# CliMA/OrthogonalSphericalShellGrids.jl

Measured on AMD Instinct MI355X. Metric: grid-cells/s metric precompute + zipper halo-fill GB/s, 1/10°×75z, higher is better.
Workload: dtype f64

## Files before the change

### orthogonalsphericalshellgrids.jl_amd/csrc/tpg_grid.hip

```cpp
#include "tpg_common.hpp"
#include "tpg_math.hpp"
#include "tpg_batch.hpp"

using namespace tpgm;

namespace {

constexpr double kC180Pi = 180.0 / kPi;
constexpr double kC360Pi = 360.0 / kPi;

struct GridK {
    int Nx, Ny, Hx, Hy;
    int shift;
    int jstart, jend;
    int jm_lo, jm_hi;
    int sx, rows;
    int ft;
    double fplp90;
    double R;
    const double* ti;
    const double* tj;
    const double* ts;
};

struct OutPtrs { void* p[TPG_NUM_ARRAYS]; };

struct TableArgs {
    int Nx, Ny, Hy, shift, ft;
    double south, npl, R;
    double* ti; double* tj; double* ts;
};

__device__ double lambda_face(int i, int N, int ft)
{
    long long num = 360ll * (i - 1) - 180ll * N;
    if (ft == TPG_F32) return (double)((float)num / (float)N);
    return (double)num / (double)N;
}
__device__ double lambda_center(int i, int N, int ft)
{
    long long num = 360ll * (2ll * i - 1) - 360ll * N;
    if (ft == TPG_F32) return (double)((float)num / (float)(2ll * N));
    return (double)num / (double)(2ll * N);
}
__device__ double phi_center(int j, int N, double south)
{
    if (N == 1) return south;
    if (south == __builtin_rint(south) && absD(south) < 1e6) {
        long long s = (long long)south;
        long long num = s * (N - 1) + (90 - s) * (long long)(j - 1);
        return (double)num / (double)(N - 1);
    }
    dd step = dd_div(two_sum(90.0, -south), dd{ (double)(N - 1), 0.0 });
    dd v = dd_add(dd{ south, 0.0 }, dd_mul_d(step, (double)(j - 1)));
    return v.hi + v.lo;
}

__global__ __launch_bounds__(64) void k_tables(TableArgs t)
{
    int tid = blockIdx.x * blockDim.x + threadIdx.x;
    const double a = tand((90.0 - t.npl) / 2);
    if (tid < t.Nx) {
        int is = tid + 1;
        int i0 = is - t.shift; if (i0 < 1) i0 += t.Nx;
        double lf = lambda_face(i0, t.Nx, t.ft), lc = lambda_center(i0, t.Nx, t.ft);
        double slf = sind(lf), clf = cosd(lf), slc = sind(lc), clc = cosd(lc);
        if (t.ft == TPG_F32) {
            slf = (double)(float)slf; clf = (double)(float)clf; slc = (double)(float)slc; clc = (double)(float)clc;
        }
        t.ti[0 * t.Nx + tid] = a * slf;
        t.ti[1 * t.Nx + tid] = a * clf;
        t.ti[2 * t.Nx + tid] = a * slc;
        t.ti[3 * t.Nx + tid] = a * clc;
        return;
    }
    tid -= t.Nx;
    if (tid < 2 * t.Ny) {
        int face = tid < t.Ny;
        int j = (face ? tid : tid - t.Ny) + 1;
        double pc = phi_center(j, t.Ny, t.south);
        double phi = pc;
        if (face) {
            double dphi = t.Ny > 1 ? phi_center(2, t.Ny, t.south) - phi_center(1, t.Ny, t.south) : 0.0;
            phi = pc - dphi / 2;
        }
        double psi = asinhD(tand((90.0 - phi) / 2) / a);
        double sh, ch;
        sinh_cosh(psi, sh, ch);
        int base = face ? 0 : 2;
        t.tj[(base + 0) * t.Ny + (j - 1)] = sh;
        t.tj[(base + 1) * t.Ny + (j - 1)] = ch;
        return;
    }
    tid -= 2 * t.Ny;
    if (tid <= t.Hy) {
        int j = 1 - t.Hy + tid;
        const double south = t.south, R = t.R;
        const double dlam = 360.0 / (double)t.Nx;
        const double dphiL = (90.0 - south) / (double)t.Ny;
        double pf, pfn, pc, pcm;
        if (south == __builtin_rint(south)) {
            long long s = (long long)south, Ny = t.Ny;
            pf  = (double)(s * Ny + (90 - s) * (long long)(j - 1)) / (double)Ny;
            pfn = (double)(s * Ny + (90 - s) * (long long)j) / (double)Ny;
            pc  = (double)(2 * s * Ny + (90 - s) * (long long)(2 * j - 1)) / (double)(2 * Ny);
            pcm = (double)(2 * s * Ny + (90 - s) * (long long)(2 * j - 3)) / (double)(2 * Ny);
        } else {
            pf  = south + (double)(j - 1) * dphiL;
            pfn = south + (double)j * dphiL;
            pc  = south + ((double)(2 * j - 1) * (90.0 - south)) / (double)(2 * t.Ny);
            pcm = south + ((double)(2 * j - 3) * (90.0 - south)) / (double)(2 * t.Ny);
        }
        int n = t.Hy + 1;
        t.ts[0 * n + tid] = R * (dlam * kDeg2Rad) * cosD(kPi * pc / 180);
        t.ts[1 * n + tid] = R * (dlam * kDeg2Rad) * cosD(kPi * pf / 180);
        t.ts[2 * n + tid] = R * R * (dlam * kDeg2Rad) * (sinD(kPi * pfn / 180) - sinD(kPi * pf / 180));
        t.ts[3 * n + tid] = R * R * (dlam * kDeg2Rad) * (sinD(kPi * pc / 180) - sinD(kPi * pcm / 180));
        t.ts[4 * n + tid] = R * (dphiL * kDeg2Rad);
    }
}

struct LP { double lam, phi; };

__device__ __forceinline__ LP analytic(const GridK& g, int xl, int yl, int is, int js)
{
    int i0 = is - g.shift; if (i0 < 1) i0 += g.Nx;
    const double* ti = g.ti + (xl == TPG_FACE ? 0 : 2) * g.Nx;
    const double* tj = g.tj + (yl == TPG_FACE ? 0 : 2) * g.Ny;
    double asl = ti[is - 1], acl = ti[g.Nx + is - 1];
    double sh = tj[js - 1], ch = tj[g.Ny + js - 1];
    double x = asl * ch;
    double y = acl * sh;
    bool pole = (x == 0.0) & (y == 0.0);
    double l = pole ? (i0 == 1 ? -90.0 : 90.0) : -kC180Pi * atanD(y / x);
    LP r;
    r.phi = 90.0 - kC360Pi * atanD(sqrt(y * y + x * x));
    l += (i0 <= g.Nx / 2) ? -90.0 : 90.0;
    l += g.fplp90;
    r.lam = fmod360(fmod360(l) + 360.0);
    return r;
}

__device__ __forceinline__ int fold_partner(int xl, int i, int Nx)
{
    int ip = (xl == TPG_FACE) ? Nx - i + 2 : Nx - i + 1;
    return ip > Nx ? ip - Nx : ip;
}

__device__ __forceinline__ LP coord(const GridK& g, int xl, int yl, int i, int j)
{
    if (j < 1) return LP{ 0.0, 0.0 };
    int iw = i < 1 ? i + g.Nx : (i > g.Nx ? i - g.Nx : i);
    int js = j;
    if (j > g.Ny) {
        int dj = j - g.Ny;
        js = (yl == TPG_FACE) ? g.Ny - dj + 1 : g.Ny - dj;
        iw = fold_partner(xl, iw, g.Nx);
        if (js < 1) return LP{ 0.0, 0.0 };
    } else if (j == g.Ny && yl == TPG_CENTER && iw > g.Nx / 2) {
        iw = fold_partner(xl, iw, g.Nx);
    }
    return analytic(g, xl, yl, iw, js);
}

__device__ __forceinline__ double haversine(LP a, LP b, double R)
{
    double dl = (b.lam - a.lam) * kDeg2Rad;
    double a1 = a.phi * kDeg2Rad;
    double a2 = b.phi * kDeg2Rad;
    double dp = a2 - a1;
    double s1 = sinD(dp / 2), s2 = sinD(dl / 2);
    double h = s1 * s1 + cosD(a1) * cosD(a2) * (s2 * s2);
    double r = sqrt(h);
    return 2 * (R * asinD(r != r ? r : (r < 1.0 ? r : 1.0)));
}

struct V3 { double x, y, z; };
__device__ __forceinline__ V3 cartesian(LP p)
{
    double cl = cosd(p.phi);
    return V3{ cosd(p.lam) * cl, sind(p.lam) * cl, sind(p.phi) };
}
__device__ __forceinline__ double dot3(V3 a, V3 b) { return a.x * b.x + a.y * b.y + a.z * b.z; }
__device__ __forceinline__ V3 cross3(V3 a, V3 b)
{
    return V3{ a.y * b.z - a.z * b.y, a.z * b.x - a.x * b.z, a.x * b.y - a.y * b.x };
}
__device__ __forceinline__ double tri_area(V3 a, V3 b, V3 c)
{
    double t = absD(dot3(a, cross3(b, c)));
    t /= 1 + dot3(a, b) + dot3(b, c) + dot3(a, c);
    return 2 * atanD(t);
}
__device__ __forceinline__ double quad_area(V3 a, V3 b, V3 c, V3 d)
{
    double A = tri_area(a, b, c);
    A += tri_area(a, b, d);
    A += tri_area(a, c, d);
    A += tri_area(b, c, d);
    return A / 2;
}

__device__ __forceinline__ double tri_tan_nr(V3 a, V3 b, V3 c)
{
    return div_nr(absD(dot3(a, cross3(b, c))), 1 + dot3(a, b) + dot3(b, c) + dot3(a, c));
}
__device__ __forceinline__ double tri_tan(V3 a, V3 b, V3 c)
{
    return absD(dot3(a, cross3(b, c))) / (1 + dot3(a, b) + dot3(b, c) + dot3(a, c));
}

template <typename T, bool NT = false>
__device__ __forceinline__ void put(const OutPtrs& o, int q, long long off, double v)
{
    T* p = static_cast<T*>(o.p[q]) + off;
    if (NT) __builtin_nontemporal_store((T)v, p); else *p = (T)v;
}

template <typename T, bool NT = false>
__device__ __forceinline__ void put32(const OutPtrs& o, int q, unsigned boff, double v)
{
    asm volatile("" : "+v"(boff));
    T* p = reinterpret_cast<T*>(static_cast<char*>(o.p[q]) + boff);
    if (NT) __builtin_nontemporal_store((T)v, p); else *p = (T)v;
}

template <typename T, bool NT>
__global__ __launch_bounds__(256) void k_cells(GridK g, OutPtrs o)
{
    const int nbx = (g.Nx + 255) / 256;
    int rb = blockIdx.x / nbx;
    int i = (blockIdx.x - rb * nbx) * 256 + threadIdx.x + 1;
    int j = g.jm_lo + rb;
    if (i > g.Nx) return;

    LP cc = coord(g, 0, 0, i, j), fc = coord(g, 1, 0, i, j), cf = coord(g, 0, 1, i, j), ff = coord(g, 1, 1, i, j);
    LP fc_e = coord(g, 1, 0, i + 1, j), fc_s = coord(g, 1, 0, i, j - 1);
    LP cc_w = coord(g, 0, 0, i - 1, j), cc_s = coord(g, 0, 0, i, j - 1), cc_sw = coord(g, 0, 0, i - 1, j - 1);
    LP ff_e = coord(g, 1, 1, i + 1, j), ff_n = coord(g, 1, 1, i, j + 1), ff_ne = coord(g, 1, 1, i + 1, j + 1);
    LP cf_w = coord(g, 0, 1, i - 1, j), cf_n = coord(g, 0, 1, i, j + 1);

    const double R = g.R;
    double dxcc = haversine(fc_e, fc, R);
    double dxfc = haversine(cc, cc_w, R);
    double dxcf = haversine(ff_e, ff, R);
    double dxff = haversine(cf, cf_w, R);
    double dycc = haversine(cf_n, cf, R);
    double dyfc = haversine(ff_n, ff, R);
    double dycf = haversine(cc, cc_s, R);
    double dyff = haversine(fc, fc_s, R);
    double azcc = quad_area(cartesian(ff), cartesian(ff_e), cartesian(ff_ne), cartesian(ff_n)) * (R * R);
    double azfc = dyfc * dxfc;
    double azcf = dycf * dxcf;
    double azff = quad_area(cartesian(cc_sw), cartesian(cc_s), cartesian(cc), cartesian(cc_w)) * (R * R);

    long long off = (long long)(i + g.Hx - 1) + (long long)g.sx * (j - g.jstart + g.Hy);
    put<T, NT>(o, TPG_LAMBDA_CC, off, cc.lam); put<T, NT>(o, TPG_LAMBDA_FC, off, fc.lam);
    put<T, NT>(o, TPG_LAMBDA_CF, off, cf.lam); put<T, NT>(o, TPG_LAMBDA_FF, off, ff.lam);
    put<T, NT>(o, TPG_PHI_CC, off, cc.phi); put<T, NT>(o, TPG_PHI_FC, off, fc.phi);
    put<T, NT>(o, TPG_PHI_CF, off, cf.phi); put<T, NT>(o, TPG_PHI_FF, off, ff.phi);
    put<T, NT>(o, TPG_DX_CC, off, dxcc); put<T, NT>(o, TPG_DX_FC, off, dxfc);
    put<T, NT>(o, TPG_DX_CF, off, dxcf); put<T, NT>(o, TPG_DX_FF, off, dxff);
    put<T, NT>(o, TPG_DY_CC, off, dycc); put<T, NT>(o, TPG_DY_CF, off, dycf);
    put<T, NT>(o, TPG_DY_FC, off, dyfc); put<T, NT>(o, TPG_DY_FF, off, dyff);
    put<T, NT>(o, TPG_AZ_CC, off, azcc); put<T, NT>(o, TPG_AZ_FC, off, azfc);
    put<T, NT>(o, TPG_AZ_CF, off, azcf); put<T, NT>(o, TPG_AZ_FF, off, azff);
}

struct Pt  { double lam, phi, a, ca; };
struct PtX { double lam, phi, a, ca, X, Y, Z; };
struct Nb  { double lam, a, ca; };
struct NbX { double lam, a, ca, X, Y, Z; };

__device__ __forceinline__ Pt make_pt(const GridK& g, int xl, int yl, int i, int j)
{
    LP p = coord(g, xl, yl, i, j);
    Pt r; r.lam = p.lam; r.phi = p.phi; r.a = p.phi * kDeg2Rad; r.ca = cosD(r.a);
    return r;
}
__device__ __forceinline__ PtX make_ptx(const GridK& g, int xl, int yl, int i, int j)
{
    LP p = coord(g, xl, yl, i, j);
    PtX r; r.lam = p.lam; r.phi = p.phi; r.a = p.phi * kDeg2Rad; r.ca = cosD(r.a);
    double sl, cl, sp, cp;
    sincosd(p.lam, sl, cl);
    sincosd(p.phi, sp, cp);
    r.X = cl * cp; r.Y = sl * cp; r.Z = sp;
    return r;
}
__device__ __forceinline__ Nb nb_of(const Pt& p) { return Nb{ p.lam, p.a, p.ca }; }
__device__ __forceinline__ Nb nb_of(const PtX& p) { return Nb{ p.lam, p.a, p.ca }; }
__device__ __forceinline__ NbX nbx_of(const PtX& p) { return NbX{ p.lam, p.a, p.ca, p.X, p.Y, p.Z }; }
__device__ __forceinline__ V3 v3_of(const PtX& p) { return V3{ p.X, p.Y, p.Z }; }
__device__ __forceinline__ V3 v3_of(const NbX& p) { return V3{ p.X, p.Y, p.Z }; }

template <int DIR> __device__ __forceinline__ double shf(double v)
{
    return DIR > 0 ? __shfl_down(v, 1, 64) : __shfl_up(v, 1, 64);
}
template <int DIR> __device__ __forceinline__ Nb shf_nb(const Pt& p)
{
    return Nb{ shf<DIR>(p.lam), shf<DIR>(p.a), shf<DIR>(p.ca) };
}
template <int DIR> __device__ __forceinline__ NbX shf_nbx(const PtX& p)
{
    return NbX{ shf<DIR>(p.lam), shf<DIR>(p.a), shf<DIR>(p.ca), shf<DIR>(p.X), shf<DIR>(p.Y), shf<DIR>(p.Z) };
}

__device__ __forceinline__ double hav(double xlam, double xa, double xca, double ylam, double ya, double yca, double R)
{
    double dl = (ylam - xlam) * kDeg2Rad;
    double dp = ya - xa;
    double s1 = sinD(dp / 2), s2 = sinD(dl / 2);
    double h = s1 * s1 + xca * yca * (s2 * s2);
    double r = sqrt(h);
    return 2 * (R * asinD(r != r ? r : (r < 1.0 ? r : 1.0)));
}
#define HAV(P, Q) hav((P).lam, (P).a, (P).ca, (Q).lam, (Q).a, (Q).ca, R)


struct Step4 {
    double lam[4], phi[4], a[4], ca[4];
    double X[2], Y[2], Z[2];
};

struct LaneConst { double aslF, aclF, aslC, aclC, hemi; };

struct RowTab { double shC, chC, shF, chF; };

typedef const double __attribute__((address_space(4))) kconst_double;
__device__ __forceinline__ RowTab load_rowtab(const GridK& g, int jc, int jf)
{
    kconst_double* tj = (kconst_double*)g.tj;
    jc = __builtin_amdgcn_readfirstlane(jc < 1 ? 1 : (jc > g.Ny ? g.Ny : jc));
    jf = __builtin_amdgcn_readfirstlane(jf < 1 ? 1 : (jf > g.Ny ? g.Ny : jf));
    return RowTab{ tj[2 * g.Ny + jc - 1], tj[3 * g.Ny + jc - 1], tj[0 * g.Ny + jf - 1], tj[1 * g.Ny + jf - 1] };
}

__device__ __forceinline__ void points_fast(const GridK& g, const LaneConst& lc, const RowTab& rt, Step4& s, const double* atab)
{
    const double shC = rt.shC, chC = rt.chC, shF = rt.shF, chF = rt.chF;
    double x[4] = { lc.aslF * chC, lc.aslC * chC, lc.aslF * chF, lc.aslC * chF };
    double y[4] = { lc.aclF * shC, lc.aclC * shC, lc.aclF * shF, lc.aclC * shF };
    double q[4], rr[4], at1[4], at2[4];
#pragma unroll
    for (int k = 0; k < 4; ++k) { q[k] = y[k] / x[k]; rr[k] = sqrt_nr<true>(y[k] * y[k] + x[k] * x[k]);    }
    tpgb::atan_tab_b<4>(q, at1, atab);
    tpgb::atan_tab_b<4, true>(rr, at2, atab);
#pragma unroll
    for (int k = 0; k < 4; ++k) {
        double l = -kC180Pi * at1[k];
        s.phi[k] = 90.0 - kC360Pi * at2[k];
        l += lc.hemi;
        l += g.fplp90;
        s.lam[k] = tpgb::fmod360_pos(tpgb::fmod360_small(l) + 360.0);
        s.a[k] = s.phi[k] * kDeg2Rad;
    }
    if (tpgb::cos_b<4>(s.a, s.ca)) {
#pragma unroll
        for (int k = 0; k < 4; ++k) s.ca[k] = cosD(s.a[k]);
    }
    double ang[4] = { s.lam[1], s.phi[1], s.lam[2], s.phi[2] }, sn[4], cs[4];
    tpgb::sincosd_b<4>(ang, sn, cs);
    s.X[0] = cs[0] * cs[1]; s.Y[0] = sn[0] * cs[1]; s.Z[0] = sn[1];
    s.X[1] = cs[2] * cs[3]; s.Y[1] = sn[2] * cs[3]; s.Z[1] = sn[3];
}

__device__ __forceinline__ void points_fast2(const GridK& g, const LaneConst& lc, const RowTab& rt, Step4& s, const double* atab)
{
    const double shC = rt.shC, chC = rt.chC, shF = rt.shF, chF = rt.chF;
    double x[4] = { lc.aslF * chC, lc.aslC * chC, lc.aslF * chF, lc.aslC * chF };
    double y[4] = { lc.aclF * shC, lc.aclC * shC, lc.aclF * shF, lc.aclC * shF };
    double q[4], rr[4], at1[4], at2[4];
    bool zerox = false;
#pragma unroll
    for (int k = 0; k < 4; ++k) { q[k] = div_nr(y[k], x[k]); zerox |= x[k] == 0.0; rr[k] = sqrt_nr<true>(y[k] * y[k] + x[k] * x[k]);    }
#pragma unroll
    for (int h = 0; h < 4; h += 2) {
        double qa[2] = { q[h], q[h + 1] }, ra[2] = { rr[h], rr[h + 1] }, o1[2], o2[2];
        tpgb::atan_tab_b<2, true>(qa, o1, atab);
        tpgb::atan_tab_b<2, true>(ra, o2, atab);
        at1[h] = o1[0]; at1[h + 1] = o1[1]; at2[h] = o2[0]; at2[h + 1] = o2[1];
    }
    if (zerox) {
#pragma unroll
        for (int k = 0; k < 4; ++k)
            if (x[k] == 0.0) {
                const double qq = y[k] / x[k];
                at1[k] = (qq != qq) ? qq : csign(kPio2Hi, qq);
            }
    }
#pragma unroll
    for (int k = 0; k < 4; ++k) {
        double l = -kC180Pi * at1[k];
        s.phi[k] = 90.0 - kC360Pi * at2[k];
        l += lc.hemi;
        l += g.fplp90;
        s.lam[k] = tpgb::fmod360_pos(tpgb::fmod360_small(l) + 360.0);
        s.a[k] = s.phi[k] * kDeg2Rad;
    }
    double sn[4], cs[4];
#pragma unroll
    for (int h = 0; h < 4; h += 2) {
        double aa[2] = { s.a[h], s.a[h + 1] }, cc2[2];
        if (tpgb::cos_lat_b<2>(aa, cc2)) { cc2[0] = cosD(aa[0]); cc2[1] = cosD(aa[1]); }
        s.ca[h] = cc2[0]; s.ca[h + 1] = cc2[1];
    }
    {
        double lon[2] = { s.lam[1], s.lam[2] }, lat[2] = { s.phi[1], s.phi[2] }, sl[2], cl[2], sp[2], cp[2];
        tpgb::sincosd_b<2>(lon, sl, cl);
        if (tpgb::sincosd_lat_b<2>(lat, sp, cp)) tpgb::sincosd_b<2>(lat, sp, cp);
        sn[0] = sl[0]; cs[0] = cl[0]; sn[1] = sp[0]; cs[1] = cp[0];
        sn[2] = sl[1]; cs[2] = cl[1]; sn[3] = sp[1]; cs[3] = cp[1];
    }
    s.X[0] = cs[0] * cs[1]; s.Y[0] = sn[0] * cs[1]; s.Z[0] = sn[1];
    s.X[1] = cs[2] * cs[3]; s.Y[1] = sn[2] * cs[3]; s.Z[1] = sn[3];
}

__device__ __noinline__ void points_general(const GridK& g, int i, int jc, int jf, Step4& s)
{
    Pt fc = make_pt(g, 1, 0, i, jc), cf = make_pt(g, 0, 1, i, jf);
    PtX cc = make_ptx(g, 0, 0, i, jc), ff = make_ptx(g, 1, 1, i, jf);
    s.lam[0] = fc.lam; s.phi[0] = fc.phi; s.a[0] = fc.a; s.ca[0] = fc.ca;
    s.lam[1] = cc.lam; s.phi[1] = cc.phi; s.a[1] = cc.a; s.ca[1] = cc.ca;
    s.lam[2] = ff.lam; s.phi[2] = ff.phi; s.a[2] = ff.a; s.ca[2] = ff.ca;
    s.lam[3] = cf.lam; s.phi[3] = cf.phi; s.a[3] = cf.a; s.ca[3] = cf.ca;
    s.X[0] = cc.X; s.Y[0] = cc.Y; s.Z[0] = cc.Z;
    s.X[1] = ff.X; s.Y[1] = ff.Y; s.Z[1] = ff.Z;
}

template <int R> struct TileLds { double v[18][R][64]; };
enum { L_FC = 0, L_CC = 3, L_FF = 9, L_CF = 15 };

template <int N>
__device__ __forceinline__ void hav_batch(const Nb (&X)[N], const Nb (&Y)[N], double Rad, double (&d)[N])
{
    double hp[N], hl[N], s1[N], s2[N], hh[N], rt[N], rm[N], as[N];
    bool zero = false;
#pragma unroll
    for (int e = 0; e < N; ++e) {
        double dp = Y[e].a - X[e].a;
        hp[e] = dp / 2; hl[e] = (Y[e].lam - X[e].lam) * (kDeg2Rad * 0.5);
    }
    if (tpgb::sin_small_b<N>(hp, s1)) {
#pragma unroll
        for (int e = 0; e < N; ++e) s1[e] = sinD(hp[e]);
    }
    if (tpgb::sin_small_b<N>(hl, s2)) {
#pragma unroll
        for (int e = 0; e < N; ++e) s2[e] = sinD(hl[e]);
    }
#pragma unroll
    for (int e = 0; e < N; ++e) {
        double h = s1[e] * s1[e] + X[e].ca * Y[e].ca * (s2[e] * s2[e]);
        hh[e] = h;
        zero |= h == 0.0;
        rt[e] = sqrt_nr<true>(h);
    }
    if (zero) {
#pragma unroll
        for (int e = 0; e < N; ++e) rt[e] = sqrt_nr(hh[e]);
    }
#pragma unroll
    for (int e = 0; e < N; ++e) {
        rm[e] = __builtin_fmin(rt[e], 1.0);
    }
    if (tpgb::asin_small_b<N>(rm, as)) {
#pragma unroll
        for (int e = 0; e < N; ++e) as[e] = asinD(!(rt[e] >= 1.0) ? rt[e] : 1.0);
    }
#pragma unroll
    for (int e = 0; e < N; ++e) d[e] = (2 * Rad) * as[e];
}

template <typename T, bool NT, int R>
__global__ __launch_bounds__(64 * R, 4) void k_cells_tile(GridK g, OutPtrs o, int tiles_x)
{
    __shared__ __attribute__((aligned(16))) double atabs[R][TPG_ATAN_TABLE_DOUBLES];
    __shared__ TileLds<R> lds;
    const int lane = threadIdx.x & 63;
    const int p = __builtin_amdgcn_readfirstlane(threadIdx.x >> 6);
    double* atab = atabs[p];
    tpgb::atan_table_init(atab, lane);
    __builtin_amdgcn_fence(__ATOMIC_RELEASE, "wavefront");
    __builtin_amdgcn_wave_barrier();
    __builtin_amdgcn_fence(__ATOMIC_ACQUIRE, "wavefront");
    const int ty = (int)gridDim.y - 1 - (int)blockIdx.y;
    const int tx = blockIdx.x;
    const int s0 = g.jm_lo - 1 + ty * (R - 1);
    const int s = s0 + p;
    int i = tx * 62 + lane;
    const bool col_emit = lane >= 1 && lane <= 62 && i <= g.Nx;
    if (i > g.Nx + 1) i = g.Nx + 1;
    const double Rad = g.R;
    const bool active_row = s <= g.jm_hi;
    const unsigned col = (unsigned)(i + g.Hx - 1);
    auto rowoff = [&](int j) -> unsigned { return (col + (unsigned)g.sx * (unsigned)(j - g.jstart + g.Hy)) * (unsigned)sizeof(T); };

    Step4 q;
    if (active_row) {
        const bool fast = s >= 1 && s < g.Ny && absD(g.fplp90) <= 360.0;
        if (fast) {
            LaneConst lc;
            const int iw = i < 1 ? i + g.Nx : (i > g.Nx ? i - g.Nx : i);
            int i0 = iw - g.shift; if (i0 < 1) i0 += g.Nx;
            lc.aslF = g.ti[0 * g.Nx + iw - 1]; lc.aclF = g.ti[1 * g.Nx + iw - 1];
            lc.aslC = g.ti[2 * g.Nx + iw - 1]; lc.aclC = g.ti[3 * g.Nx + iw - 1];
            lc.hemi = (i0 <= g.Nx / 2) ? -90.0 : 90.0;
            points_fast2(g, lc, load_rowtab(g, s, s + 1), q, atab);
        } else {
            Step4 tmp; GridK gc = g; points_general(gc, i, s, s + 1, tmp); q = tmp;
        }
        if (col_emit) {
            if (p >= 1 && s >= g.jm_lo) {
                unsigned off = rowoff(s);
                put32<T, NT>(o, TPG_LAMBDA_FC, off, q.lam[0]); put32<T, NT>(o, TPG_PHI_FC, off, q.phi[0]);
                put32<T, NT>(o, TPG_LAMBDA_CC, off, q.lam[1]); put32<T, NT>(o, TPG_PHI_CC, off, q.phi[1]);
            }
            if ((p >= 1 || ty == 0) && s + 1 >= g.jm_lo && s + 1 <= g.jm_hi) {
                unsigned off1 = rowoff(s + 1);
                put32<T, NT>(o, TPG_LAMBDA_FF, off1, q.lam[2]); put32<T, NT>(o, TPG_PHI_FF, off1, q.phi[2]);
                put32<T, NT>(o, TPG_LAMBDA_CF, off1, q.lam[3]); put32<T, NT>(o, TPG_PHI_CF, off1, q.phi[3]);
            }
        }
        double (*L)[R][64] = lds.v;
        L[L_FC + 0][p][lane] = q.lam[0]; L[L_FC + 1][p][lane] = q.a[0]; L[L_FC + 2][p][lane] = q.ca[0];
        L[L_CC + 0][p][lane] = q.lam[1]; L[L_CC + 1][p][lane] = q.a[1]; L[L_CC + 2][p][lane] = q.ca[1];
        L[L_CC + 3][p][lane] = q.X[0];   L[L_CC + 4][p][lane] = q.Y[0]; L[L_CC + 5][p][lane] = q.Z[0];
        L[L_FF + 0][p][lane] = q.lam[2]; L[L_FF + 1][p][lane] = q.a[2]; L[L_FF + 2][p][lane] = q.ca[2];
        L[L_FF + 3][p][lane] = q.X[1];   L[L_FF + 4][p][lane] = q.Y[1]; L[L_FF + 5][p][lane] = q.Z[1];
        L[L_CF + 0][p][lane] = q.lam[3]; L[L_CF + 1][p][lane] = q.a[3]; L[L_CF + 2][p][lane] = q.ca[3];
    }
    __syncthreads();
    if (p == 0) {
        if (!col_emit) return;
        double (*L)[R][64] = lds.v;
#pragma unroll 1
        for (int r = 1; r < R; r += 2) {
            const int sa = s0 + r, sb = sa + 1;
            if (sa > g.jm_hi) break;
            const bool two = (r + 1 < R) && sb <= g.jm_hi;
            const int rb = two ? r + 1 : r;
            Nb X[2] = { Nb{ L[L_FC + 0][r][lane], L[L_FC + 1][r][lane], L[L_FC + 2][r][lane] },
                        Nb{ L[L_FC + 0][rb][lane], L[L_FC + 1][rb][lane], L[L_FC + 2][rb][lane] } };
            Nb Y[2] = { Nb{ L[L_FC + 0][r - 1][lane], L[L_FC + 1][r - 1][lane], L[L_FC + 2][r - 1][lane] },
                        Nb{ L[L_FC + 0][rb - 1][lane], L[L_FC + 1][rb - 1][lane], L[L_FC + 2][rb - 1][lane] } };
            double dd2[2];
            hav_batch<2>(X, Y, Rad, dd2);
            if (sa >= g.jm_lo) put32<T, NT>(o, TPG_DY_FF, rowoff(sa), dd2[0]);
            if (two && sb >= g.jm_lo) put32<T, NT>(o, TPG_DY_FF, rowoff(sb), dd2[1]);
        }
        return;
    }
    if (!active_row || s < g.jm_lo || !col_emit) return;

    double (*L)[R][64] = lds.v;
    const int pm = p - 1, le = lane + 1, lw = lane - 1;
    const unsigned off = rowoff(s);

#pragma unroll
    for (int k = 0; k < 2; ++k) {
        V3 a, b, c, dd;
        if (k == 0) {
            a = V3{ L[L_FF + 3][pm][lane], L[L_FF + 4][pm][lane], L[L_FF + 5][pm][lane] };
            b = V3{ L[L_FF + 3][pm][le], L[L_FF + 4][pm][le], L[L_FF + 5][pm][le] };
            c = V3{ L[L_FF + 3][p][le], L[L_FF + 4][p][le], L[L_FF + 5][p][le] };
            dd = V3{ q.X[1], q.Y[1], q.Z[1] };
        } else {
            a = V3{ L[L_CC + 3][pm][lw], L[L_CC + 4][pm][lw], L[L_CC + 5][pm][lw] };
            b = V3{ L[L_CC + 3][pm][lane], L[L_CC + 4][pm][lane], L[L_CC + 5][pm][lane] };
            c = V3{ q.X[0], q.Y[0], q.Z[0] };
            dd = V3{ L[L_CC + 3][p][lw], L[L_CC + 4][p][lw], L[L_CC + 5][p][lw] };
        }
        double tt[4], at[4];
        tt[0] = tri_tan_nr(a, b, c); tt[1] = tri_tan_nr(a, b, dd);
        tt[2] = tri_tan_nr(a, c, dd); tt[3] = tri_tan_nr(b, c, dd);
        if (__any(tpgb::atan_small_b<4>(tt, at))) {
            tt[0] = tri_tan(a, b, c); tt[1] = tri_tan(a, b, dd); tt[2] = tri_tan(a, c, dd); tt[3] = tri_tan(b, c, dd);
            tpgb::atan_b<4>(tt, at);
        }
        double A = at[0];
        A += at[1];
        A += at[2];
        A += at[3];
        put32<T, NT>(o, k == 0 ? TPG_AZ_CC : TPG_AZ_FF, off, A * (Rad * Rad));
    }

    auto ld = [&](int f, int pp, int ll) -> Nb { return Nb{ L[f + 0][pp][ll], L[f + 1][pp][ll], L[f + 2][pp][ll] }; };
    const Nb own[4] = { Nb{ q.lam[0], q.a[0], q.ca[0] }, Nb{ q.lam[1], q.a[1], q.ca[1] },
                        Nb{ q.lam[2], q.a[2], q.ca[2] }, Nb{ q.lam[3], q.a[3], q.ca[3] } };
    double d[8];
#pragma unroll
    for (int hb = 0; hb < 6; hb += 2) {
        Nb X[2], Y[2];
        if (hb == 0)      { X[0] = ld(L_FC, p, le); Y[0] = own[0];            X[1] = own[1];            Y[1] = ld(L_CC, p, lw); }
        else if (hb == 2) { X[0] = ld(L_FF, pm, le); Y[0] = ld(L_FF, pm, lane); X[1] = ld(L_CF, pm, lane); Y[1] = ld(L_CF, pm, lw); }
        else              { X[0] = own[3];           Y[0] = ld(L_CF, pm, lane); X[1] = own[2];            Y[1] = ld(L_FF, pm, lane); }
        double dd2[2];
        hav_batch<2>(X, Y, Rad, dd2);
        d[hb] = dd2[0]; d[hb + 1] = dd2[1];
    }
    {
        Nb X[1] = { own[1] }, Y[1] = { ld(L_CC, pm, lane) };
        double dd1[1];
        hav_batch<1>(X, Y, Rad, dd1);
        d[6] = dd1[0];
    }
    put32<T, NT>(o, TPG_DX_CC, off, d[0]); put32<T, NT>(o, TPG_DX_FC, off, d[1]);
    put32<T, NT>(o, TPG_DX_CF, off, d[2]); put32<T, NT>(o, TPG_DX_FF, off, d[3]);
    put32<T, NT>(o, TPG_DY_CC, off, d[4]); put32<T, NT>(o, TPG_DY_FC, off, d[5]);
    put32<T, NT>(o, TPG_DY_CF, off, d[6]);
    put32<T, NT>(o, TPG_AZ_FC, off, d[5] * d[1]);
    put32<T, NT>(o, TPG_AZ_CF, off, d[6] * d[2]);
}

__device__ __forceinline__ void array_loc(int q, int& xl, int& yl)
{
    int r = q & 3;
    bool dy = (q >= TPG_DY_CC && q <= TPG_DY_FF);
    int xr = dy ? (r >> 1) : (r & 1);
    int yr = dy ? (r & 1) : (r >> 1);
    xl = xr; yl = yr;
}

struct HaloRegions {
    int nA;
    int nB;
    int nC;
    int nD;
    int nsouth;
    int merged_south;
};

template <typename T>
__global__ __launch_bounds__(256) void k_halos(GridK g, OutPtrs o, HaloRegions h)
{
    int t = blockIdx.x * blockDim.x + threadIdx.x;
    int q = blockIdx.y;
    int xl, yl;
    array_loc(q, xl, yl);
    const bool is_coord = q < TPG_DX_CC;
    T* A = static_cast<T*>(o.p[q]);
    const long long sx = g.sx;
    auto at = [&](int i, int j) -> long long { return (long long)(i + g.Hx - 1) + sx * (j - g.jstart + g.Hy); };

    int i, j;
    if (t < h.nA) {
        int r = t / (2 * g.Hx), c = t - r * 2 * g.Hx;
        j = g.jm_lo + r;
        i = c < g.Hx ? 1 - g.Hx + c : g.Nx + 1 + (c - g.Hx);
        if (h.merged_south && !is_coord && j <= 1) return;
    } else if ((t -= h.nA) < h.nB) {
        int r = t / g.sx, c = t - r * g.sx;
        j = g.Ny + 1 + r; i = 1 - g.Hx + c;
    } else if ((t -= h.nB) < h.nC) {
        int r = t / g.sx, c = t - r * g.sx;
        j = 1 - h.nsouth + r; i = 1 - g.Hx + c;
        if (is_coord) { if (j < 1) A[at(i, j)] = (T)0; return; }
        if (!h.merged_south) return;
        const int n = g.Hy + 1, rt = j - (1 - g.Hy);
        const int col = (q >= TPG_DY_CC && q <= TPG_DY_FF) ? 4 : ((q >= TPG_AZ_CC ? 2 : 0) + (yl == TPG_FACE ? 1 : 0));
        A[at(i, j)] = (T)g.ts[col * n + rt];
        return;
    } else if ((t -= h.nC) < h.nD) {
        if (is_coord || yl != TPG_CENTER) return;
        i = g.Nx / 2 + 1 + t; j = g.Ny;
    } else {
        return;
    }

    int iw = i < 1 ? i + g.Nx : (i > g.Nx ? i - g.Nx : i);
    int js = j;
    if (j > g.Ny) {
        int dj = j - g.Ny;
        js = (yl == TPG_FACE) ? g.Ny - dj + 1 : g.Ny - dj;
        iw = fold_partner(xl, iw, g.Nx);
        if (js < 1) { A[at(i, j)] = (T)0; return; }
    } else if (j == g.Ny && yl == TPG_CENTER && iw > g.Nx / 2) {
        iw = fold_partner(xl, iw, g.Nx);
    }
    A[at(i, j)] = A[at(iw, js)];
}

template <typename T>
__global__ __launch_bounds__(256) void k_south(GridK g, OutPtrs o)
{
    int c = blockIdx.x * blockDim.x + threadIdx.x;
    int r = blockIdx.y;
    int lr = (1 - g.Hy + r) - (g.jstart - g.Hy);
    if (c >= g.sx || lr < 0 || lr >= g.rows) return;
    int n = g.Hy + 1;
    double dxc = g.ts[0 * n + r], dxf = g.ts[1 * n + r], azc = g.ts[2 * n + r], azf = g.ts[3 * n + r], dy = g.ts[4 * n + r];
    long long off = (long long)c + (long long)g.sx * lr;
    put<T>(o, TPG_DX_FF, off, dxf); put<T>(o, TPG_DX_FC, off, dxc); put<T>(o, TPG_DX_CF, off, dxf); put<T>(o, TPG_DX_CC, off, dxc);
    put<T>(o, TPG_DY_FF, off, dy);  put<T>(o, TPG_DY_FC, off, dy);  put<T>(o, TPG_DY_CF, off, dy);  put<T>(o, TPG_DY_CC, off, dy);
    put<T>(o, TPG_AZ_FF, off, azf); put<T>(o, TPG_AZ_FC, off, azc); put<T>(o, TPG_AZ_CF, off, azf); put<T>(o, TPG_AZ_CC, off, azc);
}

size_t table_doubles(const tpg_params* p) { return 4 * (size_t)p->Nx + 4 * (size_t)p->Ny + 5 * (size_t)(p->Hy + 1); }

int check_params(const tpg_params* p)
{
    if (!p) { tpg::set_error("null params"); return TPG_ERR_INVALID_ARGUMENT; }
    int rc = tpg::check_geom(p->Nx, p->Ny, p->Nz, p->Hx, p->Hy, p->Hz, p->ft);
    if (rc) return rc;
    if (p->jstart < 1 || p->jend > p->Ny || p->jend < p->jstart) {
        tpg::set_error("latitude band %d:%d outside 1:%d", p->jstart, p->jend, p->Ny);
        return TPG_ERR_BAD_PARTITION;
    }
    if (p->reserved & ~TPG_BUILD_TABLES_VALID) {
        tpg::set_error("tpg_params.reserved: unknown flag bits 0x%x", p->reserved & ~TPG_BUILD_TABLES_VALID);
        return TPG_ERR_INVALID_ARGUMENT;
    }
    if (!(p->radius > 0) || !(p->north_poles_latitude < 90) || !(p->southernmost_latitude < 90)) {
        tpg::set_error("invalid radius / latitudes");
        return TPG_ERR_INVALID_ARGUMENT;
    }
    return TPG_OK;
}

template <typename T>
int launch_build(const GridK& g, const OutPtrs& o, const HaloRegions& h, hipStream_t s)
{
    dim3 grid1(((g.Nx + 255) / 256) * (g.jm_hi - g.jm_lo + 1));
    const tpg::Config& cfg = tpg::config();
    const bool nt = cfg.build_nt;
    constexpr int R = 8;
    const int nrows = g.jm_hi - g.jm_lo + 1;
    const int tiles_y = (nrows + (R - 1) - 1) / (R - 1);
    const bool offsets32 = (unsigned long long)g.sx * (unsigned long long)(g.jend - g.jstart + 1 + 2 * g.Hy) * sizeof(T) < (1ull << 32);
    const bool south_in_band = g.jstart - g.Hy <= 1;
    const bool tile = cfg.cells_variant != 0 && tiles_y <= 65535 && offsets32;
    if (tile) {
        const int tiles_x = (g.Nx + 61) / 62;
        dim3 gridt((unsigned)tiles_x, (unsigned)tiles_y);
        if (nt) hipLaunchKernelGGL((k_cells_tile<T, true, R>), gridt, dim3(64 * R), 0, s, g, o, tiles_x);
        else    hipLaunchKernelGGL((k_cells_tile<T, false, R>), gridt, dim3(64 * R), 0, s, g, o, tiles_x);
    }
    else if (nt) hipLaunchKernelGGL((k_cells<T, true>), grid1, dim3(256), 0, s, g, o);
    else         hipLaunchKernelGGL((k_cells<T, false>), grid1, dim3(256), 0, s, g, o);
    int rc = tpg::launch_status("k_cells");
    if (rc) return rc;
    HaloRegions hm = h;
    hm.merged_south = (south_in_band && g.Ny > 2 * g.Hy + 2) ? 1 : 0;
    if (hm.merged_south) hm.nC = (h.nsouth + 1) * g.sx;
    int nh = hm.nA + hm.nB + hm.nC + hm.nD;
    if (nh > 0) {
        hipLaunchKernelGGL(k_halos<T>, dim3((nh + 255) / 256, TPG_NUM_ARRAYS), dim3(256), 0, s, g, o, hm);
        if ((rc = tpg::launch_status("k_halos"))) return rc;
    }
    if (south_in_band && !hm.merged_south) {
        hipLaunchKernelGGL(k_south<T>, dim3((g.sx + 255) / 256, g.Hy + 1), dim3(256), 0, s, g, o);
        if ((rc = tpg::launch_status("k_south"))) return rc;
    }
    return TPG_OK;
}

}

extern "C" {

size_t tpg_build_grid_workspace_bytes(const tpg_params* p)
{
    if (!p || p->Nx < 1 || p->Ny < 1 || p->Hy < 0) return 0;
    return (table_doubles(p) * sizeof(double) + 255) & ~(size_t)255;
}

int tpg_build_grid(const tpg_params* p, void* const out[TPG_NUM_ARRAYS], void* workspace,
                   size_t workspace_bytes, void* stream)
{
    int rc = check_params(p);
    if (rc) return rc;
    if (!out) { tpg::set_error("null output table"); return TPG_ERR_INVALID_ARGUMENT; }
    OutPtrs o;
    for (int q = 0; q < TPG_NUM_ARRAYS; ++q) {
        if (!out[q]) { tpg::set_error("null output array %d", q); return TPG_ERR_INVALID_ARGUMENT; }
        o.p[q] = out[q];
    }
    if (!workspace || workspace_bytes < table_doubles(p) * sizeof(double) || ((uintptr_t)workspace & 7)) {
        tpg::set_error("workspace: need %zu bytes, 8-byte aligned", table_doubles(p) * sizeof(double));
        return TPG_ERR_WORKSPACE;
    }
    hipStream_t s = tpg::as_stream(stream);
    double* w = static_cast<double*>(workspace);

    TableArgs t;
    t.Nx = p->Nx; t.Ny = p->Ny; t.Hy = p->Hy; t.shift = p->Nx / 4; t.ft = p->ft;
    t.south = p->southernmost_latitude; t.npl = p->north_poles_latitude; t.R = p->radius;
    t.ti = w; t.tj = w + 4 * (size_t)p->Nx; t.ts = t.tj + 4 * (size_t)p->Ny;
    if (!(p->reserved & TPG_BUILD_TABLES_VALID)) {
        int nt = p->Nx + 2 * p->Ny + p->Hy + 1;
        hipLaunchKernelGGL(k_tables, dim3((nt + 63) / 64), dim3(64), 0, s, t);
        if ((rc = tpg::launch_status("k_tables"))) return rc;
    }

    GridK g;
    g.Nx = p->Nx; g.Ny = p->Ny; g.Hx = p->Hx; g.Hy = p->Hy; g.shift = p->Nx / 4;
    g.jstart = p->jstart; g.jend = p->jend;
    g.jm_lo = p->jstart - p->Hy < 1 ? 1 : p->jstart - p->Hy;
    g.jm_hi = p->jend + p->Hy > p->Ny ? p->Ny : p->jend + p->Hy;
    g.sx = p->Nx + 2 * p->Hx; g.rows = p->jend - p->jstart + 1 + 2 * p->Hy;
    g.ft = p->ft; g.fplp90 = p->first_pole_longitude + 90.0; g.R = p->radius;
    g.ti = t.ti; g.tj = t.tj; g.ts = t.ts;

    HaloRegions h;
    h.nA = (g.jm_hi - g.jm_lo + 1) * 2 * g.Hx;
    h.nB = (p->jend + p->Hy > p->Ny) ? (p->jend + p->Hy - p->Ny) * g.sx : 0;
    h.nsouth = (1 - (p->jstart - p->Hy)) > 0 ? (1 - (p->jstart - p->Hy)) : 0;
    h.nC = h.nsouth * g.sx;
    h.nD = (p->jend + p->Hy >= p->Ny) ? p->Nx / 2 : 0;

    if (p->ft == TPG_F64) return launch_build<double>(g, o, h, s);
    return launch_build<float>(g, o, h, s);
}

}
```

Before: 12.26 billion.

## Exploit tripolar grid mirror symmetry to halve atan and sincos work via wave shuffles

The tile kernel now assigns the lower half-wave to columns starting at a0 and the upper half-wave to the mirrored columns across the fold. Each lane computes the atan, cos and sincos for only its own row (C or F) and obtains the other row's values from its mirror lane via __shfl, with a sign fix on the longitude atan. The grid now covers only half of Nx. This roughly halves the expensive transcendental work per point, at the cost of shuffles, more complex indexing and wrapping, extra LDS reads, and reliance on the grid being exactly symmetric.

```diff
diff --git a/orthogonalsphericalshellgrids.jl_amd/csrc/tpg_grid.hip b/orthogonalsphericalshellgrids.jl_amd/csrc/tpg_grid.hip
--- a/orthogonalsphericalshellgrids.jl_amd/csrc/tpg_grid.hip
+++ b/orthogonalsphericalshellgrids.jl_amd/csrc/tpg_grid.hip
@@ -324,7 +324,7 @@
     double X[2], Y[2], Z[2];
 };
 
-struct LaneConst { double aslF, aclF, aslC, aclC, hemi; };
+struct LaneConst { double aslF, aclF, aslC, aclC, hemiF, hemiC; };
 
 struct RowTab { double shC, chC, shF, chF; };
 
@@ -337,90 +337,73 @@
     return RowTab{ tj[2 * g.Ny + jc - 1], tj[3 * g.Ny + jc - 1], tj[0 * g.Ny + jf - 1], tj[1 * g.Ny + jf - 1] };
 }
 
-__device__ __forceinline__ void points_fast(const GridK& g, const LaneConst& lc, const RowTab& rt, Step4& s, const double* atab)
-{
-    const double shC = rt.shC, chC = rt.chC, shF = rt.shF, chF = rt.chF;
-    double x[4] = { lc.aslF * chC, lc.aslC * chC, lc.aslF * chF, lc.aslC * chF };
-    double y[4] = { lc.aclF * shC, lc.aclC * shC, lc.aclF * shF, lc.aclC * shF };
-    double q[4], rr[4], at1[4], at2[4];
-#pragma unroll
-    for (int k = 0; k < 4; ++k) { q[k] = y[k] / x[k]; rr[k] = sqrt_nr<true>(y[k] * y[k] + x[k] * x[k]);    }
-    tpgb::atan_tab_b<4>(q, at1, atab);
-    tpgb::atan_tab_b<4, true>(rr, at2, atab);
+__device__ __forceinline__ double wave_mirror(double v, int plane) { return __shfl(v, plane, 64); }
+
+__device__ __forceinline__ void points_pair(const GridK& g, const LaneConst& lc, const RowTab& rt, bool upper, int plane, Step4& s, const double* atab)
+{
+    const double shS = upper ? rt.shF : rt.shC, chS = upper ? rt.chF : rt.chC;
+    const double shO = upper ? rt.shC : rt.shF, chO = upper ? rt.chC : rt.chF;
+    const double xs[2] = { lc.aslF * chS, lc.aslC * chS }, ys[2] = { lc.aclF * shS, lc.aclC * shS };
+    const double xo[2] = { lc.aslF * chO, lc.aslC * chO }, yo[2] = { lc.aclF * shO, lc.aclC * shO };
+    double qa[2], ra[2], at1s[2], at2s[2];
+    bool zerox = false;
+#pragma unroll
+    for (int c = 0; c < 2; ++c) {
+        qa[c] = div_nr(ys[c], xs[c]); zerox |= (xs[c] == 0.0) | (xo[c] == 0.0);
+        ra[c] = sqrt_nr<true>(ys[c] * ys[c] + xs[c] * xs[c]);
+    }
+    tpgb::atan_tab_b<2, true>(qa, at1s, atab);
+    tpgb::atan_tab_b<2, true>(ra, at2s, atab);
+    double phis[2], as[2], cas[2];
+#pragma unroll
+    for (int c = 0; c < 2; ++c) { phis[c] = 90.0 - kC360Pi * at2s[c]; as[c] = phis[c] * kDeg2Rad; }
+    if (tpgb::cos_lat_b<2>(as, cas)) { cas[0] = cosD(as[0]); cas[1] = cosD(as[1]); }
+    double latx[1] = { upper ? phis[0] : phis[1] }, spx[1], cpx[1];
+    if (tpgb::sincosd_lat_b<1>(latx, spx, cpx)) tpgb::sincosd_b<1>(latx, spx, cpx);
+
+    double at1o[2], phio[2], cao[2];
+#pragma unroll
+    for (int c = 0; c < 2; ++c) {
+        const double m = wave_mirror(at1s[c], plane);
+        at1o[c] = csign(m, __hiloint2double(__double2hiint(xo[c]) ^ __double2hiint(yo[c]), 0));
+        phio[c] = wave_mirror(phis[c], plane);
+        cao[c] = wave_mirror(cas[c], plane);
+    }
+    const double spo = wave_mirror(spx[0], plane), cpo = wave_mirror(cpx[0], plane);
+    if (zerox) {
+#pragma unroll
+        for (int c = 0; c < 2; ++c) {
+            if (xs[c] == 0.0) { const double qq = ys[c] / xs[c]; at1s[c] = (qq != qq) ? qq : csign(kPio2Hi, qq); }
+            if (xo[c] == 0.0) { const double qq = yo[c] / xo[c]; at1o[c] = (qq != qq) ? qq : csign(kPio2Hi, qq); }
+        }
+    }
+    double at1[4];
+#pragma unroll
+    for (int c = 0; c < 2; ++c) {
+        at1[c] = upper ? at1o[c] : at1s[c];     at1[c + 2] = upper ? at1s[c] : at1o[c];
+        s.phi[c] = upper ? phio[c] : phis[c];   s.phi[c + 2] = upper ? phis[c] : phio[c];
+        s.ca[c] = upper ? cao[c] : cas[c];      s.ca[c + 2] = upper ? cas[c] : cao[c];
+    }
 #pragma unroll
     for (int k = 0; k < 4; ++k) {
         double l = -kC180Pi * at1[k];
-        s.phi[k] = 90.0 - kC360Pi * at2[k];
-        l += lc.hemi;
+        l += (k & 1) ? lc.hemiC : lc.hemiF;
         l += g.fplp90;
         s.lam[k] = tpgb::fmod360_pos(tpgb::fmod360_small(l) + 360.0);
         s.a[k] = s.phi[k] * kDeg2Rad;
     }
-    if (tpgb::cos_b<4>(s.a, s.ca)) {
-#pragma unroll
-        for (int k = 0; k < 4; ++k) s.ca[k] = cosD(s.a[k]);
-    }
-    double ang[4] = { s.lam[1], s.phi[1], s.lam[2], s.phi[2] }, sn[4], cs[4];
-    tpgb::sincosd_b<4>(ang, sn, cs);
-    s.X[0] = cs[0] * cs[1]; s.Y[0] = sn[0] * cs[1]; s.Z[0] = sn[1];
-    s.X[1] = cs[2] * cs[3]; s.Y[1] = sn[2] * cs[3]; s.Z[1] = sn[3];
-}
-
-__device__ __forceinline__ void points_fast2(const GridK& g, const LaneConst& lc, const RowTab& rt, Step4& s, const double* atab)
-{
-    const double shC = rt.shC, chC = rt.chC, shF = rt.shF, chF = rt.chF;
-    double x[4] = { lc.aslF * chC, lc.aslC * chC, lc.aslF * chF, lc.aslC * chF };
-    double y[4] = { lc.aclF * shC, lc.aclC * shC, lc.aclF * shF, lc.aclC * shF };
-    double q[4], rr[4], at1[4], at2[4];
-    bool zerox = false;
-#pragma unroll
-    for (int k = 0; k < 4; ++k) { q[k] = div_nr(y[k], x[k]); zerox |= x[k] == 0.0; rr[k] = sqrt_nr<true>(y[k] * y[k] + x[k] * x[k]);    }
-#pragma unroll
-    for (int h = 0; h < 4; h += 2) {
-        double qa[2] = { q[h], q[h + 1] }, ra[2] = { rr[h], rr[h + 1] }, o1[2], o2[2];
-        tpgb::atan_tab_b<2, true>(qa, o1, atab);
-        tpgb::atan_tab_b<2, true>(ra, o2, atab);
-        at1[h] = o1[0]; at1[h + 1] = o1[1]; at2[h] = o2[0]; at2[h + 1] = o2[1];
-    }
-    if (zerox) {
-#pragma unroll
-        for (int k = 0; k < 4; ++k)
-            if (x[k] == 0.0) {
-                const double qq = y[k] / x[k];
-                at1[k] = (qq != qq) ? qq : csign(kPio2Hi, qq);
-            }
-    }
-#pragma unroll
-    for (int k = 0; k < 4; ++k) {
-        double l = -kC180Pi * at1[k];
-        s.phi[k] = 90.0 - kC360Pi * at2[k];
-        l += lc.hemi;
-        l += g.fplp90;
-        s.lam[k] = tpgb::fmod360_pos(tpgb::fmod360_small(l) + 360.0);
-        s.a[k] = s.phi[k] * kDeg2Rad;
-    }
-    double sn[4], cs[4];
-#pragma unroll
-    for (int h = 0; h < 4; h += 2) {
-        double aa[2] = { s.a[h], s.a[h + 1] }, cc2[2];
-        if (tpgb::cos_lat_b<2>(aa, cc2)) { cc2[0] = cosD(aa[0]); cc2[1] = cosD(aa[1]); }
-        s.ca[h] = cc2[0]; s.ca[h + 1] = cc2[1];
-    }
-    {
-        double lon[2] = { s.lam[1], s.lam[2] }, lat[2] = { s.phi[1], s.phi[2] }, sl[2], cl[2], sp[2], cp[2];
-        tpgb::sincosd_b<2>(lon, sl, cl);
-        if (tpgb::sincosd_lat_b<2>(lat, sp, cp)) tpgb::sincosd_b<2>(lat, sp, cp);
-        sn[0] = sl[0]; cs[0] = cl[0]; sn[1] = sp[0]; cs[1] = cp[0];
-        sn[2] = sl[1]; cs[2] = cl[1]; sn[3] = sp[1]; cs[3] = cp[1];
-    }
-    s.X[0] = cs[0] * cs[1]; s.Y[0] = sn[0] * cs[1]; s.Z[0] = sn[1];
-    s.X[1] = cs[2] * cs[3]; s.Y[1] = sn[2] * cs[3]; s.Z[1] = sn[3];
-}
-
-__device__ __noinline__ void points_general(const GridK& g, int i, int jc, int jf, Step4& s)
-{
-    Pt fc = make_pt(g, 1, 0, i, jc), cf = make_pt(g, 0, 1, i, jf);
-    PtX cc = make_ptx(g, 0, 0, i, jc), ff = make_ptx(g, 1, 1, i, jf);
+    double lon[2] = { s.lam[1], s.lam[2] }, sl[2], cl[2];
+    tpgb::sincosd_b<2>(lon, sl, cl);
+    const double spC = upper ? spo : spx[0], cpC = upper ? cpo : cpx[0];
+    const double spF = upper ? spx[0] : spo, cpF = upper ? cpx[0] : cpo;
+    s.X[0] = cl[0] * cpC; s.Y[0] = sl[0] * cpC; s.Z[0] = spC;
+    s.X[1] = cl[1] * cpF; s.Y[1] = sl[1] * cpF; s.Z[1] = spF;
+}
+
+__device__ __noinline__ void points_general(const GridK& g, int iF, int iC, int jc, int jf, Step4& s)
+{
+    Pt fc = make_pt(g, 1, 0, iF, jc), cf = make_pt(g, 0, 1, iC, jf);
+    PtX cc = make_ptx(g, 0, 0, iC, jc), ff = make_ptx(g, 1, 1, iF, jf);
     s.lam[0] = fc.lam; s.phi[0] = fc.phi; s.a[0] = fc.a; s.ca[0] = fc.ca;
     s.lam[1] = cc.lam; s.phi[1] = cc.phi; s.a[1] = cc.a; s.ca[1] = cc.ca;
     s.lam[2] = ff.lam; s.phi[2] = ff.phi; s.a[2] = ff.a; s.ca[2] = ff.ca;
@@ -431,6 +414,7 @@
 
 template <int R> struct TileLds { double v[18][R][64]; };
 enum { L_FC = 0, L_CC = 3, L_FF = 9, L_CF = 15 };
+enum { TILE_ADV = 30 };
 
 template <int N>
 __device__ __forceinline__ void hav_batch(const Nb (&X)[N], const Nb (&Y)[N], double Rad, double (&d)[N])
@@ -489,39 +473,50 @@
     const int tx = blockIdx.x;
     const int s0 = g.jm_lo - 1 + ty * (R - 1);
     const int s = s0 + p;
-    int i = tx * 62 + lane;
-    const bool col_emit = lane >= 1 && lane <= 62 && i <= g.Nx;
-    if (i > g.Nx + 1) i = g.Nx + 1;
+    const int Nx = g.Nx;
+    const bool upper = lane >= 32;
+    const int m = lane & 31, plane = 63 - lane;
+    const int a0 = tx * TILE_ADV;
+    const int baseA = (g.shift + a0) % Nx;
+    int baseB = (Nx + g.shift - a0 - TILE_ADV) % Nx; if (baseB < 0) baseB += Nx;
+    const bool wide = Nx >= 2 * TILE_ADV;
+    auto wrap1 = [&](int c) -> int {
+        if (wide) { c = c > Nx ? c - Nx : c; return c < 1 ? c + Nx : c; }
+        return (c + Nx - 1) % Nx + 1;
+    };
+    const int iC = wrap1((upper ? baseB : baseA) + m);
+    const int iF = upper ? wrap1(baseB + m + 1) : iC;
+    const int half = Nx >> 1;
+    const bool emitC = upper ? (m >= 1 && a0 + 31 - m <= half) : (m >= 1 && m <= TILE_ADV && a0 + m <= half);
+    const bool emitF = upper ? (m <= 30 && a0 + 30 - m <= half) : emitC;
     const double Rad = g.R;
     const bool active_row = s <= g.jm_hi;
-    const unsigned col = (unsigned)(i + g.Hx - 1);
-    auto rowoff = [&](int j) -> unsigned { return (col + (unsigned)g.sx * (unsigned)(j - g.jstart + g.Hy)) * (unsigned)sizeof(T); };
+    const unsigned colC = (unsigned)(iC + g.Hx - 1), colF = (unsigned)(iF + g.Hx - 1);
+    auto rowoffC = [&](int j) -> unsigned { return (colC + (unsigned)g.sx * (unsigned)(j - g.jstart + g.Hy)) * (unsigned)sizeof(T); };
+    auto rowoffF = [&](int j) -> unsigned { return (colF + (unsigned)g.sx * (unsigned)(j - g.jstart + g.Hy)) * (unsigned)sizeof(T); };
 
     Step4 q;
     if (active_row) {
         const bool fast = s >= 1 && s < g.Ny && absD(g.fplp90) <= 360.0;
         if (fast) {
             LaneConst lc;
-            const int iw = i < 1 ? i + g.Nx : (i > g.Nx ? i - g.Nx : i);
-            int i0 = iw - g.shift; if (i0 < 1) i0 += g.Nx;
-            lc.aslF = g.ti[0 * g.Nx + iw - 1]; lc.aclF = g.ti[1 * g.Nx + iw - 1];
-            lc.aslC = g.ti[2 * g.Nx + iw - 1]; lc.aclC = g.ti[3 * g.Nx + iw - 1];
-            lc.hemi = (i0 <= g.Nx / 2) ? -90.0 : 90.0;
-            points_fast2(g, lc, load_rowtab(g, s, s + 1), q, atab);
+            int i0F = iF - g.shift; if (i0F < 1) i0F += Nx;
+            int i0C = iC - g.shift; if (i0C < 1) i0C += Nx;
+            lc.aslF = g.ti[0 * Nx + iF - 1]; lc.aclF = g.ti[1 * Nx + iF - 1];
+            lc.aslC = g.ti[2 * Nx + iC - 1]; lc.aclC = g.ti[3 * Nx + iC - 1];
+            lc.hemiF = (i0F <= half) ? -90.0 : 90.0;
+            lc.hemiC = (i0C <= half) ? -90.0 : 90.0;
+            points_pair(g, lc, load_rowtab(g, s, s + 1), upper, plane, q, atab);
         } else {
-            Step4 tmp; GridK gc = g; points_general(gc, i, s, s + 1, tmp); q = tmp;
-        }
-        if (col_emit) {
-            if (p >= 1 && s >= g.jm_lo) {
-                unsigned off = rowoff(s);
-                put32<T, NT>(o, TPG_LAMBDA_FC, off, q.lam[0]); put32<T, NT>(o, TPG_PHI_FC, off, q.phi[0]);
-                put32<T, NT>(o, TPG_LAMBDA_CC, off, q.lam[1]); put32<T, NT>(o, TPG_PHI_CC, off, q.phi[1]);
-            }
-            if ((p >= 1 || ty == 0) && s + 1 >= g.jm_lo && s + 1 <= g.jm_hi) {
-                unsigned off1 = rowoff(s + 1);
-                put32<T, NT>(o, TPG_LAMBDA_FF, off1, q.lam[2]); put32<T, NT>(o, TPG_PHI_FF, off1, q.phi[2]);
-                put32<T, NT>(o, TPG_LAMBDA_CF, off1, q.lam[3]); put32<T, NT>(o, TPG_PHI_CF, off1, q.phi[3]);
-            }
+            Step4 tmp; GridK gc = g; points_general(gc, iF, iC, s, s + 1, tmp); q = tmp;
+        }
+        if (p >= 1 && s >= g.jm_lo) {
+            if (emitF) { unsigned off = rowoffF(s); put32<T, NT>(o, TPG_LAMBDA_FC, off, q.lam[0]); put32<T, NT>(o, TPG_PHI_FC, off, q.phi[0]); }
+            if (emitC) { unsigned off = rowoffC(s); put32<T, NT>(o, TPG_LAMBDA_CC, off, q.lam[1]); put32<T, NT>(o, TPG_PHI_CC, off, q.phi[1]); }
+        }
+        if ((p >= 1 || ty == 0) && s + 1 >= g.jm_lo && s + 1 <= g.jm_hi) {
+            if (emitF) { unsigned off1 = rowoffF(s + 1); put32<T, NT>(o, TPG_LAMBDA_FF, off1, q.lam[2]); put32<T, NT>(o, TPG_PHI_FF, off1, q.phi[2]); }
+            if (emitC) { unsigned off1 = rowoffC(s + 1); put32<T, NT>(o, TPG_LAMBDA_CF, off1, q.lam[3]); put32<T, NT>(o, TPG_PHI_CF, off1, q.phi[3]); }
         }
         double (*L)[R][64] = lds.v;
         L[L_FC + 0][p][lane] = q.lam[0]; L[L_FC + 1][p][lane] = q.a[0]; L[L_FC + 2][p][lane] = q.ca[0];
@@ -533,7 +528,7 @@
     }
     __syncthreads();
     if (p == 0) {
-        if (!col_emit) return;
+        if (!emitF) return;
         double (*L)[R][64] = lds.v;
 #pragma unroll 1
         for (int r = 1; r < R; r += 2) {
@@ -547,25 +542,25 @@
                         Nb{ L[L_FC + 0][rb - 1][lane], L[L_FC + 1][rb - 1][lane], L[L_FC + 2][rb - 1][lane] } };
             double dd2[2];
             hav_batch<2>(X, Y, Rad, dd2);
-            if (sa >= g.jm_lo) put32<T, NT>(o, TPG_DY_FF, rowoff(sa), dd2[0]);
-            if (two && sb >= g.jm_lo) put32<T, NT>(o, TPG_DY_FF, rowoff(sb), dd2[1]);
+            if (sa >= g.jm_lo) put32<T, NT>(o, TPG_DY_FF, rowoffF(sa), dd2[0]);
+            if (two && sb >= g.jm_lo) put32<T, NT>(o, TPG_DY_FF, rowoffF(sb), dd2[1]);
         }
         return;
     }
-    if (!active_row || s < g.jm_lo || !col_emit) return;
+    if (!active_row || s < g.jm_lo || !emitC) return;
 
     double (*L)[R][64] = lds.v;
-    const int pm = p - 1, le = lane + 1, lw = lane - 1;
-    const unsigned off = rowoff(s);
+    const int pm = p - 1, lw = lane - 1, lf = upper ? lane - 1 : lane, le = lf + 1;
+    const unsigned off = rowoffC(s);
 
 #pragma unroll
     for (int k = 0; k < 2; ++k) {
         V3 a, b, c, dd;
         if (k == 0) {
-            a = V3{ L[L_FF + 3][pm][lane], L[L_FF + 4][pm][lane], L[L_FF + 5][pm][lane] };
+            a = V3{ L[L_FF + 3][pm][lf], L[L_FF + 4][pm][lf], L[L_FF + 5][pm][lf] };
             b = V3{ L[L_FF + 3][pm][le], L[L_FF + 4][pm][le], L[L_FF + 5][pm][le] };
             c = V3{ L[L_FF + 3][p][le], L[L_FF + 4][p][le], L[L_FF + 5][p][le] };
-            dd = V3{ q.X[1], q.Y[1], q.Z[1] };
+            dd = V3{ L[L_FF + 3][p][lf], L[L_FF + 4][p][lf], L[L_FF + 5][p][lf] };
         } else {
             a = V3{ L[L_CC + 3][pm][lw], L[L_CC + 4][pm][lw], L[L_CC + 5][pm][lw] };
             b = V3{ L[L_CC + 3][pm][lane], L[L_CC + 4][pm][lane], L[L_CC + 5][pm][lane] };
@@ -587,21 +582,20 @@
     }
 
     auto ld = [&](int f, int pp, int ll) -> Nb { return Nb{ L[f + 0][pp][ll], L[f + 1][pp][ll], L[f + 2][pp][ll] }; };
-    const Nb own[4] = { Nb{ q.lam[0], q.a[0], q.ca[0] }, Nb{ q.lam[1], q.a[1], q.ca[1] },
-                        Nb{ q.lam[2], q.a[2], q.ca[2] }, Nb{ q.lam[3], q.a[3], q.ca[3] } };
+    const Nb ownC[2] = { Nb{ q.lam[1], q.a[1], q.ca[1] }, Nb{ q.lam[3], q.a[3], q.ca[3] } };
     double d[8];
 #pragma unroll
     for (int hb = 0; hb < 6; hb += 2) {
         Nb X[2], Y[2];
-        if (hb == 0)      { X[0] = ld(L_FC, p, le); Y[0] = own[0];            X[1] = own[1];            Y[1] = ld(L_CC, p, lw); }
-        else if (hb == 2) { X[0] = ld(L_FF, pm, le); Y[0] = ld(L_FF, pm, lane); X[1] = ld(L_CF, pm, lane); Y[1] = ld(L_CF, pm, lw); }
-        else              { X[0] = own[3];           Y[0] = ld(L_CF, pm, lane); X[1] = own[2];            Y[1] = ld(L_FF, pm, lane); }
+        if (hb == 0)      { X[0] = ld(L_FC, p, le); Y[0] = ld(L_FC, p, lf);     X[1] = ownC[0];           Y[1] = ld(L_CC, p, lw); }
+        else if (hb == 2) { X[0] = ld(L_FF, pm, le); Y[0] = ld(L_FF, pm, lf);   X[1] = ld(L_CF, pm, lane); Y[1] = ld(L_CF, pm, lw); }
+        else              { X[0] = ownC[1];          Y[0] = ld(L_CF, pm, lane); X[1] = ld(L_FF, p, lf);    Y[1] = ld(L_FF, pm, lf); }
         double dd2[2];
         hav_batch<2>(X, Y, Rad, dd2);
         d[hb] = dd2[0]; d[hb + 1] = dd2[1];
     }
     {
-        Nb X[1] = { own[1] }, Y[1] = { ld(L_CC, pm, lane) };
+        Nb X[1] = { ownC[0] }, Y[1] = { ld(L_CC, pm, lane) };
         double dd1[1];
         hav_batch<1>(X, Y, Rad, dd1);
         d[6] = dd1[0];
@@ -732,7 +726,7 @@
     const bool south_in_band = g.jstart - g.Hy <= 1;
     const bool tile = cfg.cells_variant != 0 && tiles_y <= 65535 && offsets32;
     if (tile) {
-        const int tiles_x = (g.Nx + 61) / 62;
+        const int tiles_x = (g.Nx / 2 + TILE_ADV - 1) / TILE_ADV;
         dim3 gridt((unsigned)tiles_x, (unsigned)tiles_y);
         if (nt) hipLaunchKernelGGL((k_cells_tile<T, true, R>), gridt, dim3(64 * R), 0, s, g, o, tiles_x);
         else    hipLaunchKernelGGL((k_cells_tile<T, false, R>), gridt, dim3(64 * R), 0, s, g, o, tiles_x);
```

New measurement: 11.85 billion. -3.3%, worse.
